# zhirui-gao/Curve-Gaussian

Hardware: AMD Instinct MI355X
Metric: Msplats rasterized/s (fwd+bwd) (higher is better)
Workload: dtype f32

## Files before the change

curve_gaussian_amd/csrc/api.hip:

```cpp
#include <math.h>
#include <stdarg.h>
#include <stdio.h>
#include <string.h>
#include <stdlib.h>

#include <algorithm>
#include <atomic>
#include <map>
#include <mutex>
#include <string>
#include <vector>

#include "kernels.h"

namespace cgs {

static thread_local char g_err[512] = "";
void set_error(const char* fmt, ...) {
    va_list ap;
    va_start(ap, fmt);
    vsnprintf(g_err, sizeof(g_err), fmt, ap);
    va_end(ap);
}

// ... 310 lines not shown
}
static void slot_abandon(int i) {
    if (g_slots[i].in_flight) (void)hipEventSynchronize(g_slots[i].ev);
    g_slots[i].in_flight = false;
    slot_release(i);
}
static bool slot_read(int i, const uint32_t* words, hipStream_t s, const char* what) {
    hipError_t e = hipMemcpyAsync(g_slots[i].h, words, 4 * sizeof(uint32_t), hipMemcpyDeviceToHost, s);
    if (e == hipSuccess) e = hipEventRecord(g_slots[i].ev, s);
    g_slots[i].in_flight = true;
    if (e != hipSuccess) set_error("%s: status readback failed: %s", what, hipGetErrorString(e));
    return e == hipSuccess;
}
static bool slot_sync(int i, const char* what) {
    const hipError_t e = hipEventSynchronize(g_slots[i].ev);
    g_slots[i].in_flight = e != hipSuccess;
    if (e != hipSuccess) set_error("%s: status readback failed: %s", what, hipGetErrorString(e));
    return e == hipSuccess;
}
static bool slot_wait(int i, const char* what) {
    if (!slot_sync(i, what)) return false;
    const StatSlot& v = g_slots[i];
    const uint32_t longest = v.h[1];
    hints_update(v.P, v.W, v.H, (uint64_t)longest <= v.cap ? (int64_t)v.h[0] : -1, longest, (int64_t)v.h[3], v.dev);
    g_last_stats[0] = (int64_t)v.h[0]; g_last_stats[1] = (int64_t)longest; g_last_stats[2] = 1;
    g_last_visible = (int64_t)v.h[2];
    return true;
}

static bool bucket_tail(hipStream_t s, const char* what, const Frame& f, const States& b, uint64_t cap, int P, const int* radii,
                        const BinHints& hints, int cull, uint32_t* nonunit, bool geo, bool unit, bool tag,
                        const float* background, float* out_color, float* out_invdepth, float* out_all_map,
                        float* color_clamped, float* dir_out, const float* wv, int slot) {
    launch_scatter_bucket(s, P, radii, b.geom.rec, f.gx, f.gy, b.img.tile_count, b.bin.keys, (uint32_t)cap, cull, b.img.total + 3,
                          hints.big > 0 ? b.img.tile_cursor : nullptr, (uint32_t)f.tiles, nonunit, scatter_spw(hints));
    if (slot >= 0) {
        uint32_t* const stat = b.img.work + 4;
        hipLaunchKernelGGL(k_count_stats, dim3(STAT_BLOCKS), dim3(256), 0, s, b.img.tile_count, f.tiles, radii, P, b.img.total + 3,
                           stat, b.img.work + VIS_COUNT_WORD);
        if (!slot_read(slot, stat, s, what)) return false;
        StatSlot& v = g_slots[slot];
        v.P = P; v.W = f.W; v.H = f.H; v.cap = cap;
    }
    if (render_fwd_can_sort((uint32_t)cap) && fuse_sort()) {
        launch_render_fwd_sorting(s, geo, f.tiles, b.img.tile_count, b.bin.keys, (uint32_t)cap, b.img.ranges, b.img.total,
                                  b.bin.point_list, f.W, f.H, f.gx, b.geom.rec, b.img.final_T, b.img.n_contrib, background,
                                  out_color, out_invdepth, out_all_map, unit, tag, color_clamped, dir_out, wv);
    } else {
        launch_tile_sort_bucket(s, f.tiles, b.img.tile_count, b.img.ranges, b.img.total, b.bin.keys, b.bin.point_list,
                                (uint32_t)cap);
        launch_render_fwd(s, geo, f.tiles, b.img.ranges, b.bin.point_list, f.W, f.H, f.gx, b.geom.rec, b.img.final_T,
                          b.img.n_contrib, background, out_color, out_invdepth, out_all_map, unit, tag);
        if (color_clamped || dir_out)
            hipLaunchKernelGGL(k_render_epilogue, dim3((unsigned)std::min<size_t>((f.npix + 255) / 256, 4096)), dim3(256), 0, s,
                               f.npix, out_color, out_all_map, wv, 1, color_clamped, dir_out);
    }
    return check_launch(what, false, s);
}

extern "C" {

const char* cgs_last_error(void) { return g_err; }
int cgs_version(void) { return 100; }
const char* cgs_target_arch(void) { return "gfx950"; }

size_t cgs_geometry_bytes(int P) {
    char* c = nullptr;
    geom_from_chunk(c, (size_t)(P > 0 ? P : 1));
    return (size_t)c + 128;
}
size_t cgs_image_bytes(int width, int height) {
    char* c = nullptr;
    const Frame f(width, height);
    image_from_chunk(c, f.npix, (size_t)f.tiles);
    return (size_t)c + 128;
}
size_t cgs_binning_bytes(int64_t R) {
    char* c = nullptr;
    bin_from_chunk(c, (size_t)(R > 0 ? R : 1));
// ... 875 lines not shown
```

curve_gaussian_amd/csrc/binning.hip:

```cpp
#include "kernels.h"

namespace cgs {

__global__ void __launch_bounds__(1024) k_scan_tiles(int tiles, const uint32_t* __restrict__ tile_count,
                                                     uint2* __restrict__ ranges, uint32_t* __restrict__ total) {
    __shared__ uint32_t wave_tot[16];
    __shared__ uint32_t wave_max[16];
    __shared__ uint32_t carry_s;
    const int tid = threadIdx.x, lane = tid & 63, wid = tid >> 6;
    if (tid == 0) carry_s = 0;
    __syncthreads();
    uint32_t vmax = 0;
    for (int base = 0; base < tiles; base += 1024) {
        const int i = base + tid;
        const uint32_t v = (i < tiles) ? tile_count[i] : 0u;
        vmax = max(vmax, v);
        uint32_t s = v;
#pragma unroll
        for (int off = 1; off < 64; off <<= 1) {
            const uint32_t n = __shfl_up(s, off, 64);
            if (lane >= off) s += n;
        }
        if (lane == 63) wave_tot[wid] = s;
        __syncthreads();
// ... 172 lines not shown
        }
        const bool gvalid = src < 64;
        const SplatWalk sp = me.fetch(gvalid ? src : lane);
        const uint32_t nt = gvalid ? sp.nt : 0u;
        for (uint32_t base = 0; __ballot(base < nt) != 0ull; base += 16) {
            const uint32_t t = base + (uint32_t)sub;
            bool pass = false;
            uint32_t tile = 0, gx_ = 0, gy_ = 0;
            if (t < nt) {
                const uint32_t ty = t / sp.w, tx = t - ty * sp.w;
                const uint32_t gxx = sp.x0 + tx, gyy = sp.y0 + ty;
                pass = !cull || tile_reach_det(sp.cx, sp.cy, sp.A, sp.B, sp.C, sp.tau2, (float)(gxx * TILE), (float)(gyy * TILE));
                tile = gyy * (uint32_t)grid_x + gxx;
                gx_ = gxx; gy_ = gyy;
            }
            fn(pass, tile, ((uint64_t)sp.khi << 32) | sp.klo, gx_, gy_);
        }
    }
}
__device__ __forceinline__ void wave_lds_fence() {
    __builtin_amdgcn_fence(__ATOMIC_RELEASE, "wavefront");
    __builtin_amdgcn_wave_barrier();
    __builtin_amdgcn_fence(__ATOMIC_ACQUIRE, "wavefront");
}
constexpr uint32_t BIG_TILES = 96;
constexpr uint32_t GW_WIN = 16, GW_CELLS = GW_WIN * GW_WIN;
#ifndef CGS_GW_LCAP
#define CGS_GW_LCAP 192
#endif
constexpr uint32_t GW_LCAP = CGS_GW_LCAP;
template <int GW_SPW>
__global__ void __launch_bounds__(256) k_scatter_window(int P, const int* __restrict__ radii,
                                                        const SplatRec* __restrict__ rec, int grid_x, int grid_y,
                                                        uint32_t* __restrict__ tile_count, uint64_t* __restrict__ keys,
                                                        uint32_t cap, int cull, uint32_t* __restrict__ big_count,
                                                        uint32_t* __restrict__ big_queue, uint32_t big_cap,
                                                        uint32_t* __restrict__ nonunit) {
    __shared__ uint32_t s_cell[4][GW_CELLS];
    __shared__ uint16_t s_ent[4][GW_LCAP];
    __shared__ uint64_t s_key[4][GW_LCAP];
    const uint32_t lane = threadIdx.x & 63, wave = threadIdx.x >> 6;
    uint32_t* wcell = s_cell[wave];
    uint16_t* went = s_ent[wave];
    uint64_t* wkey = s_key[wave];
    const int idx = (blockIdx.x * 4 + (int)wave) * GW_SPW + (int)lane;
    SplatWalk me = load_splat_walk((int)lane < GW_SPW, idx, P, radii, rec, grid_x, grid_y);
    if (nonunit && me.nonunit) *nonunit = 1u;
    if (me.nt > BIG_TILES) {
        const uint32_t q = atomicAdd(big_count, 1u);
        if (big_queue && q < big_cap) {
            big_queue[q] = (uint32_t)idx;
            me.nt = 0u;
        }
    }
    if (__ballot(me.nt > 0) == 0ull) return;
    uint32_t wx0 = me.nt > 0 ? me.x0 : 0xFFFFFFFFu, wy0 = me.nt > 0 ? me.y0 : 0xFFFFFFFFu;
#pragma unroll
    for (int off = 32; off >= 1; off >>= 1) {
        wx0 = min(wx0, (uint32_t)__shfl_xor((int)wx0, off, 64));
        wy0 = min(wy0, (uint32_t)__shfl_xor((int)wy0, off, 64));
    }
    wx0 = (uint32_t)__builtin_amdgcn_readfirstlane((int)wx0);
    wy0 = (uint32_t)__builtin_amdgcn_readfirstlane((int)wy0);
#pragma unroll
    for (uint32_t q = 0; q < GW_CELLS / 64; q++) wcell[lane + 64 * q] = 0u;
    wave_lds_fence();
    uint32_t cnt = 0;
    quad_walk(me, grid_x, cull, [&](bool pass, uint32_t tile, uint64_t key, uint32_t gxx, uint32_t gyy) {
        const uint32_t dx = gxx - wx0, dy = gyy - wy0;
        const bool inwin = pass && dx < GW_WIN && dy < GW_WIN;
        const uint64_t bal = __ballot(inwin);
        const uint32_t pos = cnt + __builtin_amdgcn_mbcnt_hi((uint32_t)(bal >> 32), __builtin_amdgcn_mbcnt_lo((uint32_t)bal, 0u));
        if (inwin && pos < GW_LCAP) {
            const uint32_t cell = dy * GW_WIN + dx;
            const uint32_t r = atomicAdd(&wcell[cell], 1u);
            went[pos] = (uint16_t)(cell | (r << 8));
            wkey[pos] = key;
        } else if (pass) {
            const uint32_t slot = atomicAdd(&tile_count[tile], 1u);
            if (slot < cap) keys[(size_t)tile * cap + slot] = key;
        }
        cnt += (uint32_t)__builtin_popcountll(bal);
    });
    const uint32_t n = min(cnt, GW_LCAP);
    if (n == 0) return;
    wave_lds_fence();
#pragma unroll
    for (uint32_t q = 0; q < GW_CELLS / 64; q++) {
        const uint32_t cell = lane + 64 * q;
        const uint32_t c = wcell[cell];
        if (c) {
            const uint32_t tile = (wy0 + cell / GW_WIN) * (uint32_t)grid_x + wx0 + cell % GW_WIN;
            wcell[cell] = atomicAdd(&tile_count[tile], c);
        }
    }
    wave_lds_fence();
    for (uint32_t j = lane; j < n; j += 64) {
        const uint32_t e = went[j], cell = e & 255u;
        const uint32_t slot = wcell[cell] + (e >> 8);
        const uint32_t tile = (wy0 + cell / GW_WIN) * (uint32_t)grid_x + wx0 + cell % GW_WIN;
        if (slot < cap) keys[(size_t)tile * cap + slot] = wkey[j];
    }
}

__global__ void __launch_bounds__(256) k_scatter_big(const uint32_t* __restrict__ big_count,
                                                     const uint32_t* __restrict__ big_queue, uint32_t big_cap,
                                                     const int* __restrict__ radii, const SplatRec* __restrict__ rec,
                                                     int grid_x, int grid_y, uint32_t* __restrict__ tile_count,
                                                     uint64_t* __restrict__ keys, uint32_t cap, int cull) {
    const uint32_t n = min(*big_count, big_cap);
    for (uint32_t e = blockIdx.x; e < n; e += gridDim.x) {
        const int idx = (int)big_queue[e];
        const float4 a = rec[idx].a;
        const float4 d = rec[idx].d;
        const float C = rec[idx].b.x;
        uint2 rmin, rmax;
        get_rect(a.x, a.y, radii[idx], grid_x, grid_y, rmin, rmax);
        const uint32_t w = max(rmax.x - rmin.x, 1u), nt = (rmax.x - rmin.x) * (rmax.y - rmin.y);
        const uint64_t key = ((uint64_t)__float_as_uint(d.x) << 32) | (uint32_t)idx;
        for (uint32_t t = threadIdx.x; t < nt; t += 256) {
            const uint32_t ty = t / w, tx = t - ty * w;
            const uint32_t gxx = rmin.x + tx, gyy = rmin.y + ty;
            if (cull && !tile_reach_det(a.x, a.y, a.z, a.w, C, d.z, (float)(gxx * TILE), (float)(gyy * TILE))) continue;
            const uint32_t tile = gyy * (uint32_t)grid_x + gxx;
            const uint32_t slot = atomicAdd(&tile_count[tile], 1u);
            if (slot < cap) keys[(size_t)tile * cap + slot] = key;
        }
    }
}

#ifndef CGS_RANK_SPLIT
#define CGS_RANK_SPLIT 1024
#endif
constexpr uint32_t RANK_SPLIT = CGS_RANK_SPLIT;
constexpr uint32_t RANK_MAX2 = 2048;
template <bool BUCKET, int KPT, bool PUBLISH>
__global__ void __launch_bounds__(256) k_tile_rank_sort(const uint2* __restrict__ ranges,
                                                        const uint64_t* __restrict__ keys,
                                                        uint32_t* __restrict__ point_list, uint32_t cap,
                                                        const uint32_t* __restrict__ tile_count,
                                                        uint2* __restrict__ ranges_out, uint32_t* __restrict__ total,
                                                        uint32_t min_n) {
    __shared__ __attribute__((aligned(16))) uint32_t sd[256 * KPT + RANK_U];
    __shared__ uint32_t si[256 * KPT];
    __shared__ uint32_t s_hist[RANK_NB], s_start[RANK_NB + 1], s_mm[8];
    const uint2 rg = BUCKET ? bucket_range(tile_count, ranges_out, total, cap, PUBLISH) : ranges[blockIdx.x];
    const uint32_t n = rg.y - rg.x;
    if (n <= min_n || n > 256u * KPT || n > (KPT == 4 ? RANK_SPLIT : ~0u) || (!BUCKET && rg.y > cap)) return;
    const uint32_t tid = threadIdx.x;
    if ((tid & ~63u) >= n) return;
    uint32_t rank[KPT], idx[KPT];
    tile_rank_sort<KPT>(keys + rg.x, n, RankScratch{sd, si, s_hist, s_start, s_mm}, rank, idx);
    uint32_t* out = point_list + rg.x;
#pragma unroll
    for (int q = 0; q < KPT; q++) {
        const uint32_t i = tid + 256u * q;
        if (i < n) out[rank[q]] = idx[q];
    }
}
// ... 30 lines not shown


void launch_scan_tiles(hipStream_t s, int tiles, const uint32_t* tile_count, uint2* ranges, uint32_t* total) {
    ProfScope p("scan_tiles", s);
    hipLaunchKernelGGL(k_scan_tiles, dim3(1), dim3(1024), 0, s, tiles, tile_count, ranges, total);
}
void launch_scatter(hipStream_t s, int P, const int* radii, const SplatRec* rec, int grid_x, int grid_y,
                    const uint2* ranges, uint32_t* tile_cursor, uint64_t* keys, uint32_t cap, int cull, uint32_t* nonunit) {
    ProfScope p("scatter", s);
    hipLaunchKernelGGL(k_scatter<false>, dim3((P + 4 * SCATTER_SPW - 1) / (4 * SCATTER_SPW)), dim3(256), 0, s, P,
                       radii, rec, grid_x, grid_y, ranges, tile_cursor, keys, cap, cull, nonunit);
}
void launch_tile_sort_small(hipStream_t s, int tiles, const uint2* ranges, uint64_t* keys, uint32_t* point_list,
                            uint32_t cap) {
    ProfScope p("tile_sort", s);
    hipLaunchKernelGGL((k_tile_rank_sort<false, 4, false>), dim3(tiles), dim3(256), 0, s, ranges, keys, point_list, cap,
                       nullptr, nullptr, nullptr, 0u);
}
void launch_tile_sort_big(hipStream_t s, int tiles, const uint2* ranges, uint64_t* keys, uint32_t* point_list,
                          uint32_t max_count) {
    if (max_count <= RANK_SPLIT) return;
    uint32_t done = RANK_SPLIT;
    if (RANK_SPLIT == RANK_MAX) {
        ProfScope p("tile_sort_mid", s);
        hipLaunchKernelGGL((k_tile_rank_sort<false, 8, false>), dim3(tiles), dim3(256), 0, s, ranges, keys, point_list,
                           ~0u, nullptr, nullptr, nullptr, RANK_MAX);
        done = RANK_MAX2;
    }
    ProfScope p("tile_sort_big", s);
    if (max_count > done)
        hipLaunchKernelGGL(k_tile_sort<false>, dim3(tiles), dim3(256), 0, s, ranges, keys, point_list, done, 0u, nullptr);
}
void launch_scatter_bucket(hipStream_t s, int P, const int* radii, const SplatRec* rec, int grid_x, int grid_y,
                           uint32_t* tile_count, uint64_t* keys, uint32_t cap, int cull, uint32_t* big_count,
                           uint32_t* big_queue, uint32_t big_cap, uint32_t* nonunit, int splats_per_wave) {
    ProfScope p("scatter", s);
    if (splats_per_wave == 8)
        hipLaunchKernelGGL(k_scatter_window<8>, dim3((P + 4 * 8 - 1) / (4 * 8)), dim3(256), 0, s, P, radii, rec, grid_x,
                           grid_y, tile_count, keys, cap, cull, big_count, big_queue, big_cap, nonunit);
    else
        hipLaunchKernelGGL(k_scatter_window<12>, dim3((P + 4 * 12 - 1) / (4 * 12)), dim3(256), 0, s, P, radii, rec, grid_x,
                           grid_y, tile_count, keys, cap, cull, big_count, big_queue, big_cap, nonunit);
    if (big_queue)
        hipLaunchKernelGGL(k_scatter_big, dim3(512), dim3(256), 0, s, big_count, big_queue, big_cap, radii, rec, grid_x,
                           grid_y, tile_count, keys, cap, cull);
}
void launch_tile_sort_bucket(hipStream_t s, int tiles, const uint32_t* tile_count, uint2* ranges, uint32_t* total,
                             uint64_t* keys, uint32_t* point_list, uint32_t cap) {
    {
        ProfScope p("tile_sort", s);
        hipLaunchKernelGGL((k_tile_rank_sort<true, 4, true>), dim3(tiles), dim3(256), 0, s, nullptr, keys, point_list, cap,
                           tile_count, ranges, total, 0u);
    }
    if (cap > RANK_SPLIT) {
        uint32_t done = RANK_SPLIT;
        if (RANK_SPLIT == RANK_MAX) {
            ProfScope p("tile_sort_mid", s);
            hipLaunchKernelGGL((k_tile_rank_sort<true, 8, false>), dim3(tiles), dim3(256), 0, s, nullptr, keys, point_list,
                               cap, tile_count, nullptr, nullptr, RANK_MAX);
            done = RANK_MAX2;
        }
        ProfScope p("tile_sort_big", s);
        if (cap > done)
            hipLaunchKernelGGL(k_tile_sort<true>, dim3(tiles), dim3(256), 0, s, nullptr, keys, point_list, done, cap,
                               tile_count);
    }
}
uint32_t bucket_cap_limit() { return SORT_LDS_KEYS; }

}
```

curve_gaussian_amd/csrc/common.h:

```cpp
#pragma once
#include <hip/hip_runtime.h>
#include <stdint.h>

#include "../../include/curvegs.h"

namespace cgs {

constexpr int TILE = 16;
constexpr int TILE_PIX = TILE * TILE;
constexpr int NUM_ALL_MAP = 4;

struct __attribute__((aligned(64))) SplatRec {
    float4 a, b, c, d;
};

constexpr int ACC_STRIDE = 16;
constexpr int ACC_STRIDE_VIEW = 8;
constexpr int ACC_COL = 6, ACC_INVD = 7, ACC_MAP = 8;

constexpr uint32_t LIST_TAG_SHIFT = 28u;
constexpr uint32_t LIST_ID_MASK = (1u << LIST_TAG_SHIFT) - 1u;

struct GeomState {
    SplatRec* rec;
    float* grad_acc;
    float* rgb;
    uint8_t* clamped;
};
constexpr int WORK_WORDS = 64 * 32;
constexpr int TOTAL_PARTS = 256;
constexpr int TOTAL_WORDS = 4 + 2 * TOTAL_PARTS;
struct ImageState {
    float* final_T;
    uint32_t* n_contrib;
    uint2* ranges;
    uint32_t* tile_count;
    uint32_t* tile_cursor;
    uint32_t* work;
    uint32_t* total;
};
struct BinState {
    uint64_t* keys;
    uint32_t* point_list;
};

template <typename T>
static inline void carve(char*& chunk, T*& ptr, size_t count) {
    uintptr_t off = (reinterpret_cast<uintptr_t>(chunk) + 127) & ~uintptr_t(127);
    ptr = reinterpret_cast<T*>(off);
    chunk = reinterpret_cast<char*>(ptr + count);
}
static inline GeomState geom_from_chunk(char*& chunk, size_t P) {
    GeomState g;
    carve(chunk, g.rec, P);
    carve(chunk, g.grad_acc, P * ACC_STRIDE);
    carve(chunk, g.rgb, P);
    carve(chunk, g.clamped, P);
    return g;
}
static inline ImageState image_from_chunk(char*& chunk, size_t npix, size_t tiles) {
    ImageState s;
    carve(chunk, s.final_T, npix);
    carve(chunk, s.n_contrib, npix);
    carve(chunk, s.ranges, tiles);
    carve(chunk, s.tile_count, tiles);
    carve(chunk, s.tile_cursor, tiles);
    carve(chunk, s.work, WORK_WORDS);
    carve(chunk, s.total, TOTAL_WORDS + 32);
    return s;
}
static inline BinState bin_from_chunk(char*& chunk, size_t R) {
    BinState b;
    carve(chunk, b.point_list, R);
    carve(chunk, b.keys, R);
    return b;
}

#ifdef __HIPCC__
__device__ __forceinline__ float3 xform4x3(const float3 p, const float* __restrict__ m) {
#pragma clang fp contract(off)
    return make_float3(m[0] * p.x + m[4] * p.y + m[8] * p.z + m[12], m[1] * p.x + m[5] * p.y + m[9] * p.z + m[13],
                       m[2] * p.x + m[6] * p.y + m[10] * p.z + m[14]);
}
__device__ __forceinline__ float4 xform4x4(const float3 p, const float* __restrict__ m) {
#pragma clang fp contract(off)
    return make_float4(m[0] * p.x + m[4] * p.y + m[8] * p.z + m[12], m[1] * p.x + m[5] * p.y + m[9] * p.z + m[13],
                       m[2] * p.x + m[6] * p.y + m[10] * p.z + m[14], m[3] * p.x + m[7] * p.y + m[11] * p.z + m[15]);
}
__device__ __forceinline__ float ndc2pix(float v, int S) { return (float)((((double)v + 1.0) * (double)S - 1.0) * 0.5); }

__device__ __forceinline__ void get_rect(float px, float py, int max_radius, int gx, int gy, uint2& rmin, uint2& rmax) {
    rmin.x = (uint32_t)min(gx, max(0, (int)((px - (float)max_radius) / (float)TILE)));
    rmin.y = (uint32_t)min(gy, max(0, (int)((py - (float)max_radius) / (float)TILE)));
    rmax.x = (uint32_t)min(gx, max(0, (int)((px + (float)max_radius + (float)(TILE - 1)) / (float)TILE)));
    rmax.y = (uint32_t)min(gy, max(0, (int)((py + (float)max_radius + (float)(TILE - 1)) / (float)TILE)));
}

__device__ __forceinline__ void quat_rows(const float4 q, float R[3][3]) {
#pragma clang fp contract(off)
    const float r = q.x, x = q.y, y = q.z, z = q.w;
// ... 119 lines not shown
#pragma unroll
        for (int q = 0; q < NQ; q++)
#pragma unroll
            for (uint32_t e = 0; e < RANK_U; e++) rank[q] += (uint32_t)(k[e] < mine[q]);
#pragma unroll
        for (uint32_t e = 0; e < RANK_U; e++) k[e] = p[e];
    }
#pragma unroll
    for (int q = 0; q < NQ; q++)
#pragma unroll
        for (uint32_t e = 0; e < RANK_U; e++) rank[q] += (uint32_t)(k[e] < mine[q]);
}
__device__ __forceinline__ uint32_t rank_loop_f32(const float* s, uint32_t n, float mine) {
    float big = 0x1p64f, nbig = -0x1p64f;
    asm volatile("" : "+v"(big), "+v"(nbig));
    const float mb = mine * big;
    const uint32_t nu = (n + 3u) & ~3u;
    float r0 = 0.f, r1 = 0.f, r2 = 0.f, r3 = 0.f;
    float4 k = *reinterpret_cast<const float4*>(s);
    for (uint32_t u = 4; u < nu; u += 4) {
        const float4 p = *reinterpret_cast<const float4*>(s + u);
        r0 += __builtin_amdgcn_fmed3f(fmaf(k.x, nbig, mb), 0.f, 1.f);
        r1 += __builtin_amdgcn_fmed3f(fmaf(k.y, nbig, mb), 0.f, 1.f);
        r2 += __builtin_amdgcn_fmed3f(fmaf(k.z, nbig, mb), 0.f, 1.f);
        r3 += __builtin_amdgcn_fmed3f(fmaf(k.w, nbig, mb), 0.f, 1.f);
        k = p;
    }
    r0 += __builtin_amdgcn_fmed3f(fmaf(k.x, nbig, mb), 0.f, 1.f);
    r1 += __builtin_amdgcn_fmed3f(fmaf(k.y, nbig, mb), 0.f, 1.f);
    r2 += __builtin_amdgcn_fmed3f(fmaf(k.z, nbig, mb), 0.f, 1.f);
    r3 += __builtin_amdgcn_fmed3f(fmaf(k.w, nbig, mb), 0.f, 1.f);
    return (uint32_t)((r0 + r1) + (r2 + r3));
}
template <typename K>
__device__ __forceinline__ void rank_dispatch(int nq, const K* s, uint32_t n, const K (&mine)[4], uint32_t (&rank)[4]) {
    switch (nq) {
        case 1: rank_loop<1>(s, n, mine, rank); break;
        case 2: rank_loop<2>(s, n, mine, rank); break;
        case 3: rank_loop<3>(s, n, mine, rank); break;
        default: rank_loop<4>(s, n, mine, rank); break;
    }
}

#ifndef CGS_RANK_PARTITION_MIN
#define CGS_RANK_PARTITION_MIN 192
#endif
constexpr uint32_t RANK_PARTITION_MIN = CGS_RANK_PARTITION_MIN;
#ifndef CGS_RANK_NB
#define CGS_RANK_NB 64
#endif
constexpr uint32_t RANK_NB = CGS_RANK_NB;
struct RankScratch {
    uint32_t* sd;
    uint32_t* si;
    uint32_t* hist;
    uint32_t* start;
    uint32_t* mm;
};
template <int KPT>
__device__ __forceinline__ void tile_rank_sort(const uint64_t* __restrict__ gk, uint32_t n, const RankScratch S,
                                               uint32_t (&rank)[KPT], uint32_t (&idx)[KPT]) {
    const uint32_t tid = threadIdx.x;
    const int lane = (int)(tid & 63u), wave = (int)(tid >> 6);
    const bool has_keys = ((uint32_t)__builtin_amdgcn_readfirstlane((int)tid) & ~63u) < n;
    const int nq = (int)((n + 255u) / 256u);
    (void)nq;
// ... 144 lines not shown
```

curve_gaussian_amd/csrc/kernels.h:

```cpp
#pragma once
#include "common.h"

namespace cgs {

void launch_preprocess_fwd(hipStream_t s, int P, int D, int M, const float* means3D, const float* scales,
                           float scale_modifier, const float* rotations, const float* opacities, const float* shs,
                           uint8_t* clamped, const float* cov3D_precomp, const float* colors_precomp,
                           const float* all_map, const float* viewmatrix, const float* projmatrix,
                           const float* cam_pos, int W, int H, float tan_fovx, float tan_fovy, float focal_x,
                           float focal_y, int* radii, SplatRec* rec, float* rgb, int grid_x, int grid_y,
                           uint32_t* tile_count, int antialiasing, int cull, float* grad_acc, uint32_t* clear_words,
                           size_t n_clear);
void launch_mark_visible(hipStream_t s, int P, const float* means3D, const float* viewmatrix, uint8_t* present);
void launch_preprocess_bwd(hipStream_t s, int P, int D, int M, const float* means3D, const int* radii,
                           const float* shs, const uint8_t* clamped, const float* opacities, const float* scales,
                           const float* rotations, float scale_modifier, const float* cov3D_precomp,
                           const float* viewmatrix, const float* projmatrix, const float* cam_pos, float focal_x,
                           float focal_y, float tan_fovx, float tan_fovy, int W, int H, const SplatRec* rec,
                           float* grad_acc, float* dL_dmean2D, float* dL_dconic, float* dL_dinvdepth,
                           float* dL_dopacity, float* dL_dmean3D, float* dL_dcolor, float* dL_dall_map,
                           float* dL_dcov3D, float* dL_dsh, float* dL_dscale, float* dL_drot, int antialiasing);

void launch_scan_tiles(hipStream_t s, int tiles, const uint32_t* tile_count, uint2* ranges, uint32_t* total);
void launch_scatter(hipStream_t s, int P, const int* radii, const SplatRec* rec, int grid_x, int grid_y,
                    const uint2* ranges, uint32_t* tile_cursor, uint64_t* keys, uint32_t cap, int cull,
                    uint32_t* nonunit = nullptr);
void launch_scatter_bucket(hipStream_t s, int P, const int* radii, const SplatRec* rec, int grid_x, int grid_y,
                           uint32_t* tile_count, uint64_t* keys, uint32_t cap, int cull, uint32_t* big_count,
                           uint32_t* big_queue, uint32_t big_cap, uint32_t* nonunit = nullptr,
                           int splats_per_wave = 12);
void launch_tile_sort_bucket(hipStream_t s, int tiles, const uint32_t* tile_count, uint2* ranges, uint32_t* total,
                             uint64_t* keys, uint32_t* point_list, uint32_t cap);
uint32_t bucket_cap_limit();
void launch_tile_sort_small(hipStream_t s, int tiles, const uint2* ranges, uint64_t* keys, uint32_t* point_list,
                            uint32_t cap);
void launch_tile_sort_big(hipStream_t s, int tiles, const uint2* ranges, uint64_t* keys, uint32_t* point_list,
                          uint32_t max_count);

void launch_render_fwd(hipStream_t s, bool geo, int tiles, const uint2* ranges, const uint32_t* point_list, int W,
                       int H, int grid_x, const SplatRec* rec, float* final_T, uint32_t* n_contrib,
                       const float* bg_color, float* out_color, float* out_invdepth, float* out_all_map,
                       bool unit = false,
                       bool tag = false);
bool render_fwd_can_sort(uint32_t cap);
void launch_render_fwd_sorting(hipStream_t s, bool geo, int tiles, const uint32_t* tile_count, const uint64_t* keys,
                               uint32_t cap, uint2* ranges, uint32_t* total, uint32_t* point_list, int W, int H,
                               int grid_x, const SplatRec* rec, float* final_T, uint32_t* n_contrib,
                               const float* bg_color, float* out_color, float* out_invdepth, float* out_all_map,
                               bool unit = false, bool tag = false,
                               float* color_clamped = nullptr, float* dir_out = nullptr, const float* wv = nullptr);
void launch_render_bwd(hipStream_t s, bool geo, bool invd, bool colg, int tiles, const uint2* ranges,
                       const uint32_t* point_list, int W, int H, int grid_x, const float* bg_color,
                       const SplatRec* rec, const float* final_Ts, const uint32_t* n_contrib, const float* dL_dpixels,
                       const float* dL_dout_invdepth, const float* dL_dout_all_map, float* grad_acc,
                       int acc_stride = ACC_STRIDE,
                       uint32_t id_mask = 0xffffffffu,
                       const uint32_t* nonunit_gate = nullptr);


void launch_render_bwd_unit(hipStream_t s, int tiles, const uint2* ranges, const uint32_t* point_list, int W, int H,
                            int grid_x, const float* bg_color, const SplatRec* rec, const float* final_Ts,
                            const uint32_t* n_contrib, const float* dL_dpixels, float* grad_acc,
                            int acc_stride = ACC_STRIDE_VIEW, const uint32_t* nonunit_gate = nullptr,
                            const float* clamp_raw = nullptr);

int sample_norm_words();
void launch_sample_norms(hipStream_t s, int B, int m, const float* cp, const uint8_t* is_bezier, const void* coef, double* norms);
void launch_sample_backward_close(hipStream_t s, int B, int m, const float* cp, const float* width, const uint8_t* is_bezier,
                                  const void* coef, float eps, const double* norms, const float* part, float* g_cp, float* g_width,
                                  int accumulate);
void launch_view_forward(hipStream_t s, int B, int m, const float* cp, const float* width, const uint8_t* is_bezier,
                         const void* coef, float eps, const double* norms, const float* opacity_logit,
                         const float* mask_logit, float mask_thr, const float* colors_precomp, const float* campos,
                         const float* viewmatrix, const float* projmatrix, float tan_fovx, float tan_fovy, float focal_x,
                         float focal_y, int W, int H, int grid_x, int grid_y, float* xyz, float* rot, float* scl, int* radii,
                         SplatRec* rec, float* grad_acc, uint32_t* clear_words, size_t n_clear);
void launch_view_backward(hipStream_t s, int B, int m, const float* cp, const float* width, const uint8_t* is_bezier,
                          const void* coef, float eps, double* norms, const float* opacity_logit, const float* mask_logit,
// ... 60 lines not shown
```

curve_gaussian_amd/csrc/render.hip:

```cpp
#include "kernels.h"
#include "p2_mfma.h"
#include "composite.h"

namespace cgs {

constexpr int BATCH = 256;
__device__ __forceinline__ float sat01(float x) { return __builtin_amdgcn_fmed3f(x, 0.f, 1.f); }
struct StepConsts {
    float big, cA;
};
__device__ __forceinline__ StepConsts step_consts() {
    StepConsts k;
    k.big = 0x1p100f;
    k.cA = -__uint_as_float(0x3b808080u) * 0x1p100f;
    asm volatile("" : "+v"(k.big), "+v"(k.cA));
    return k;
}
constexpr int SLOTS = 8;

struct BucketSort {
    const uint32_t* tile_count;
    const uint64_t* keys;
    uint32_t* point_list;
    uint2* ranges;
    uint32_t* total;
    uint32_t cap;
};

struct ViewEpilogue {
    float* color_clamped;
    float* dir_out;
    const float* wv;
};

constexpr int GROUP = 16;
#ifndef CGS_WHATIF
#define CGS_WHATIF 0
#endif
#ifndef CGS_FWD3_WAVES
#define CGS_FWD3_WAVES 6
#endif
#ifndef CGS_FWD3_WAVES_GENERAL
#define CGS_FWD3_WAVES_GENERAL CGS_FWD3_WAVES
#endif
#ifndef CGS_FWD_FAST
#define CGS_FWD_FAST 1
#endif
#ifndef CGS_BWD3_WHATIF
#define CGS_BWD3_WHATIF 0
#endif
#ifndef CGS_BWD3_WAVES
#define CGS_BWD3_WAVES 6
#endif
#ifndef CGS_BWD3_CAP
#define CGS_BWD3_CAP 104
#endif
constexpr int BWD_BATCH = 128;
static_assert(CGS_BWD3_CAP % 8 == 0 && CGS_BWD3_CAP <= BWD_BATCH, "CGS_BWD3_CAP: a multiple of SLOTS (8), at most BWD_BATCH");
constexpr uint32_t BWD_PAD_OFF = (BWD_BATCH + 1) * 16;
constexpr uint32_t PAD_OFF = (BATCH + 1) * 16;

template <bool GEO, bool SORT, bool UNIT = false, bool TAG = UNIT>
__global__ void __launch_bounds__(256, UNIT ? CGS_FWD3_WAVES : CGS_FWD3_WAVES_GENERAL) k_render_fwd3(const uint2* __restrict__ ranges,
                                                     const uint32_t* __restrict__ point_list, int W, int H, int grid_x,
                                                     const SplatRec* __restrict__ rec, float* __restrict__ final_T,
                                                     uint32_t* __restrict__ n_contrib, const float* __restrict__ bg_color,
                                                     float* __restrict__ out_color, float* __restrict__ out_invdepth,
                                                     float* __restrict__ out_all_map, BucketSort bs, ViewEpilogue epi) {
    constexpr bool IMAGE_ONLY = UNIT && !GEO;
    __shared__ float4 s_geo[BATCH + 2];
    __shared__ float4 s_at[BATCH + 2];
    __shared__ float4 s_c[GEO ? BATCH + 2 : 1];
    __shared__ uint64_t s_qmask[4][4];
    __shared__ __attribute__((aligned(16))) uint32_t s_list[4][BATCH + GROUP];
    __shared__ __attribute__((aligned(16))) uint32_t s_ord[SORT ? RANK_MAX + RANK_U : 1];
    __shared__ uint32_t s_si[SORT ? RANK_MAX : 1];
    __shared__ uint32_t s_hist[SORT ? RANK_NB : 1], s_start[SORT ? RANK_NB + 1 : 1], s_mm[8];
    if (threadIdx.x == 0) {
        s_geo[BATCH + 1] = make_float4(0.f, 0.f, 0.f, 0.f);
        s_at[BATCH + 1] = make_float4(0.f, 0.f, 0.f, L2_NEVER);
        if (GEO) s_c[GEO ? BATCH + 1 : 0] = make_float4(0.f, 0.f, 0.f, 0.f);
    }
    const TileGeom g = tile_geom(W, H, grid_x);
    const int lane = g.lane;
    const float X0 = (float)(g.tx * TILE), Y0 = (float)(g.ty * TILE);
    uint2 range;
    bool prestaged = false;
    if (SORT) {
        const uint32_t tid = threadIdx.x;
        const uint32_t base = g.tile * bs.cap;
        uint64_t key0 = ~0ull;
        if (CGS_FWD_FAST && tid < bs.cap) key0 = bs.keys[base + tid];
        const uint32_t cnt = bs.tile_count[g.tile];
        const uint32_t n = min(cnt, bs.cap);
        range = make_uint2(base, base + n);
        if (tid == 0) {
            bs.ranges[g.tile] = range;
            if (cnt) {
                uint32_t* part = bs.total + 4 + 2 * (g.tile % TOTAL_PARTS);
                atomicAdd(&part[0], n);
                atomicMax(&part[1], cnt);
                if (cnt > bs.cap) {
                    bs.total[2] = 1u;
                    atomicAdd(&bs.total[TOTAL_WORDS], 1u);
                }
            }
        }
        if (CGS_FWD_FAST && n > 0 && n <= (uint32_t)BATCH) {
            const bool has = tid < n;
            const uint32_t depth = has ? (uint32_t)(key0 >> 32) : ~0u;
            const uint32_t id = has ? (uint32_t)key0 : 0u;
            const SplatRec* r = rec + id;
            float4 ra = make_float4(0.f, 0.f, 1.f, 0.f), rb = make_float4(1.f, 0.f, 0.f, 0.f), rc = ra;
            float tau2 = -1.f;
            if (has && !(CGS_WHATIF & 256)) {
                ra = r->a;
                rb = r->b;
                if (GEO) rc = r->c;
                tau2 = r->d.z;
            }
            if (has) s_ord[tid] = depth;
            if (tid < 4u) s_ord[n + tid] = 0x7f800000u;
            s_si[tid] = 0u;
            __syncthreads();
            uint32_t lost = 0u;
            if (((uint32_t)__builtin_amdgcn_readfirstlane((int)tid) & ~63u) < n) {
                const uint32_t rk[1] = {(CGS_WHATIF & 32) ? tid : rank_loop_f32(reinterpret_cast<const float*>(s_ord), n, __uint_as_float(depth))};
                if (has) {
                    float4 sa, sb;
                    stage_splat(ra, rb, sa, sb);
                    const uint32_t slot = rk[0] + 1u;
                    s_geo[slot] = sa;
                    s_at[slot] = make_float4(sb.z, sb.w, sb.x, __builtin_amdgcn_logf(sb.y));
                    if (GEO) s_c[GEO ? slot : 0] = UNIT ? make_float4(rc.x, rc.y, rc.z, sb.w) : rc;
                    const uint32_t qm = (CGS_WHATIF & 128) ? 15u : quadrant_mask(ra, rb, tau2, X0, Y0);
                    lost = atomicExch(&s_si[rk[0]], 0x100u | qm);
                    bs.point_list[base + rk[0]] = TAG ? (id | (qm << LIST_TAG_SHIFT)) : id;
                }
            }
            prestaged = !__syncthreads_or((int)lost);
        }
        if (n > 0 && !prestaged) {
            uint32_t rank[4], idx[4];
            tile_rank_sort<4>(bs.keys + base, n, RankScratch{s_ord, s_si, s_hist, s_start, s_mm}, rank, idx);
#pragma unroll
            for (int q = 0; q < 4; q++) {
                const uint32_t i = tid + 256u * q;
                if (i < n) {
                    s_ord[rank[q]] = idx[q];
                    if (!TAG || rank[q] >= (uint32_t)BATCH) bs.point_list[base + rank[q]] = idx[q];
                }
            }
            __syncthreads();
        }
    } else {
        range = ranges[g.tile];
    }
    const int total = (int)(range.y - range.x);
    const int rounds = (total + BATCH - 1) / BATCH;
    const StepConsts k = step_consts();
    float T_dead = 0.0f;
    float Tw = 1.0f;
    float cA = g.inside ? k.cA : -0x1p126f;
    uint32_t last_contributor = 0;
    float C = 0.f, Dacc = 0.f;
    float A0 = 0.f, A1 = 0.f, A2 = 0.f, A3 = 0.f;
    bool wave_done = ballot64(cA > -0x1p120f) == 0ull;
    const P2Frag pix = p2_pixel_operand(lane);
    const int row_splat = p2_row_splat(lane);
    const float hx = X0 + (float)((g.wave & 1) << 3) + 3.5f;
// ... 484 lines not shown
#pragma unroll
                        for (int w = 0; w < 4; w++) {
                            const uint64_t m = tm[w][c];
                            const int pos = base[w][c] + __builtin_popcountll(m & ((1ull << bit) - 1ull));
                            if (((m >> bit) & 1ull) && pos < CAP) { v += s_res[w][pos * NF + f]; any = true; }
                        }
                        if (any && v != 0.f) {
                            const uint32_t id = INVD ? s_id[e + 1] : __float_as_uint(s_at[e + 1].y);
                            atomicAdd(grad_acc + (size_t)id * acc_stride + f, v);
                        }
                    }
                }
            }
        }
    }
}

#define CGS_FWD3(G, S, U, T, R, PL, BS)                                                                               \
    hipLaunchKernelGGL((k_render_fwd3<G, S, U, T>), dim3(tiles), dim3(256), 0, s, R, PL, W, H, grid_x, rec, final_T,  \
                       n_contrib, bg_color, out_color, out_invdepth, out_all_map, BS, epi)
void launch_render_fwd(hipStream_t s, bool geo, int tiles, const uint2* ranges, const uint32_t* point_list, int W,
                       int H, int grid_x, const SplatRec* rec, float* final_T, uint32_t* n_contrib,
                       const float* bg_color, float* out_color, float* out_invdepth, float* out_all_map, bool unit, bool tag) {
    ProfScope p("render_fwd", s);
    const ViewEpilogue epi{nullptr, nullptr, nullptr};
    if (geo && unit) CGS_FWD3(true, false, true, true, ranges, point_list, BucketSort{});
    else if (unit) CGS_FWD3(false, false, true, true, ranges, point_list, BucketSort{});
    else if (geo && tag) CGS_FWD3(true, false, false, true, ranges, point_list, BucketSort{});
    else if (tag) CGS_FWD3(false, false, false, true, ranges, point_list, BucketSort{});
    else if (geo) CGS_FWD3(true, false, false, false, ranges, point_list, BucketSort{});
    else CGS_FWD3(false, false, false, false, ranges, point_list, BucketSort{});
}
bool render_fwd_can_sort(uint32_t cap) { return cap <= RANK_MAX; }
void launch_render_fwd_sorting(hipStream_t s, bool geo, int tiles, const uint32_t* tile_count, const uint64_t* keys,
                               uint32_t cap, uint2* ranges, uint32_t* total, uint32_t* point_list, int W, int H,
                               int grid_x, const SplatRec* rec, float* final_T, uint32_t* n_contrib,
                               const float* bg_color, float* out_color, float* out_invdepth, float* out_all_map, bool unit,
                               bool tag, float* color_clamped, float* dir_out, const float* wv) {
    ProfScope p("render_fwd", s);
    const BucketSort bs{tile_count, keys, point_list, ranges, total, cap};
    const ViewEpilogue epi{color_clamped, geo ? dir_out : nullptr, wv};
    const uint2* no_ranges = nullptr;
    const uint32_t* no_list = nullptr;
    if (geo && unit) CGS_FWD3(true, true, true, true, no_ranges, no_list, bs);
    else if (unit) CGS_FWD3(false, true, true, true, no_ranges, no_list, bs);
    else if (geo && tag) CGS_FWD3(true, true, false, true, no_ranges, no_list, bs);
    else if (tag) CGS_FWD3(false, true, false, true, no_ranges, no_list, bs);
    else if (geo) CGS_FWD3(true, true, false, false, no_ranges, no_list, bs);
    else CGS_FWD3(false, true, false, false, no_ranges, no_list, bs);
}
#undef CGS_FWD3
void launch_render_bwd(hipStream_t s, bool geo, bool invd, bool colg, int tiles, const uint2* ranges,
                       const uint32_t* point_list, int W, int H, int grid_x, const float* bg_color,
                       const SplatRec* rec, const float* final_Ts, const uint32_t* n_contrib, const float* dL_dpixels,
                       const float* dL_dout_invdepth, const float* dL_dout_all_map, float* grad_acc, int acc_stride,
                       uint32_t id_mask, const uint32_t* nonunit_gate) {
    ProfScope p("render_bwd", s);
#define CGS_BWD(G, I, C)                                                                                         \
    hipLaunchKernelGGL((k_render_bwd3<G, I, C>), dim3(tiles), dim3(256), 0, s, ranges, point_list, W, H, grid_x, \
                       bg_color, rec, final_Ts, n_contrib, dL_dpixels, dL_dout_invdepth, dL_dout_all_map, grad_acc, acc_stride, id_mask, nonunit_gate)
    if (geo && invd) CGS_BWD(true, true, true);
    else if (geo) CGS_BWD(true, false, true);
    else if (invd) CGS_BWD(false, true, true);
    else if (colg) CGS_BWD(false, false, true);
    else CGS_BWD(false, false, false);
#undef CGS_BWD
}

}
```

Measured before the change: 817.7.

## Bucket per-tile depth ranking into sub-ranges using scatter-tracked depth bounds

```diff
diff --git a/curve_gaussian_amd/csrc/api.hip b/curve_gaussian_amd/csrc/api.hip
--- a/curve_gaussian_amd/csrc/api.hip
+++ b/curve_gaussian_amd/csrc/api.hip
@@ -366,8 +366,9 @@
                         const BinHints& hints, int cull, uint32_t* nonunit, bool geo, bool unit, bool tag,
                         const float* background, float* out_color, float* out_invdepth, float* out_all_map,
                         float* color_clamped, float* dir_out, const float* wv, int slot) {
-    launch_scatter_bucket(s, P, radii, b.geom.rec, f.gx, f.gy, b.img.tile_count, b.bin.keys, (uint32_t)cap, cull, b.img.total + 3,
-                          hints.big > 0 ? b.img.tile_cursor : nullptr, (uint32_t)f.tiles, nonunit, scatter_spw(hints));
+    launch_scatter_bucket(s, P, radii, b.geom.rec, f.gx, f.gy, b.img.tile_count, b.img.tile_depth, b.bin.keys, (uint32_t)cap, cull,
+                          b.img.total + 3, hints.big > 0 ? b.img.tile_cursor : nullptr, (uint32_t)f.tiles, nonunit,
+                          scatter_spw(hints));
     if (slot >= 0) {
         uint32_t* const stat = b.img.work + 4;
         hipLaunchKernelGGL(k_count_stats, dim3(STAT_BLOCKS), dim3(256), 0, s, b.img.tile_count, f.tiles, radii, P, b.img.total + 3,
@@ -377,8 +378,8 @@
         v.P = P; v.W = f.W; v.H = f.H; v.cap = cap;
     }
     if (render_fwd_can_sort((uint32_t)cap) && fuse_sort()) {
-        launch_render_fwd_sorting(s, geo, f.tiles, b.img.tile_count, b.bin.keys, (uint32_t)cap, b.img.ranges, b.img.total,
-                                  b.bin.point_list, f.W, f.H, f.gx, b.geom.rec, b.img.final_T, b.img.n_contrib, background,
+        launch_render_fwd_sorting(s, geo, f.tiles, b.img.tile_count, b.img.tile_depth, b.bin.keys, (uint32_t)cap, b.img.ranges,
+                                  b.img.total, b.bin.point_list, f.W, f.H, f.gx, b.geom.rec, b.img.final_T, b.img.n_contrib, background,
                                   out_color, out_invdepth, out_all_map, unit, tag, color_clamped, dir_out, wv);
     } else {
         launch_tile_sort_bucket(s, f.tiles, b.img.tile_count, b.img.ranges, b.img.total, b.bin.keys, b.bin.point_list,
diff --git a/curve_gaussian_amd/csrc/binning.hip b/curve_gaussian_amd/csrc/binning.hip
--- a/curve_gaussian_amd/csrc/binning.hip
+++ b/curve_gaussian_amd/csrc/binning.hip
@@ -228,10 +228,10 @@
 template <int GW_SPW>
 __global__ void __launch_bounds__(256) k_scatter_window(int P, const int* __restrict__ radii,
                                                         const SplatRec* __restrict__ rec, int grid_x, int grid_y,
-                                                        uint32_t* __restrict__ tile_count, uint64_t* __restrict__ keys,
-                                                        uint32_t cap, int cull, uint32_t* __restrict__ big_count,
-                                                        uint32_t* __restrict__ big_queue, uint32_t big_cap,
-                                                        uint32_t* __restrict__ nonunit) {
+                                                        uint32_t* __restrict__ tile_count, uint2* __restrict__ tile_depth,
+                                                        uint64_t* __restrict__ keys, uint32_t cap, int cull,
+                                                        uint32_t* __restrict__ big_count, uint32_t* __restrict__ big_queue,
+                                                        uint32_t big_cap, uint32_t* __restrict__ nonunit) {
     __shared__ uint32_t s_cell[4][GW_CELLS];
     __shared__ uint16_t s_ent[4][GW_LCAP];
     __shared__ uint64_t s_key[4][GW_LCAP];
@@ -251,13 +251,18 @@
     }
     if (__ballot(me.nt > 0) == 0ull) return;
     uint32_t wx0 = me.nt > 0 ? me.x0 : 0xFFFFFFFFu, wy0 = me.nt > 0 ? me.y0 : 0xFFFFFFFFu;
+    uint32_t wlo = me.nt > 0 ? ~me.khi : 0u, whi = me.nt > 0 ? me.khi : 0u;
 #pragma unroll
     for (int off = 32; off >= 1; off >>= 1) {
         wx0 = min(wx0, (uint32_t)__shfl_xor((int)wx0, off, 64));
         wy0 = min(wy0, (uint32_t)__shfl_xor((int)wy0, off, 64));
+        wlo = max(wlo, (uint32_t)__shfl_xor((int)wlo, off, 64));
+        whi = max(whi, (uint32_t)__shfl_xor((int)whi, off, 64));
     }
     wx0 = (uint32_t)__builtin_amdgcn_readfirstlane((int)wx0);
     wy0 = (uint32_t)__builtin_amdgcn_readfirstlane((int)wy0);
+    wlo = (uint32_t)__builtin_amdgcn_readfirstlane((int)wlo);
+    whi = (uint32_t)__builtin_amdgcn_readfirstlane((int)whi);
 #pragma unroll
     for (uint32_t q = 0; q < GW_CELLS / 64; q++) wcell[lane + 64 * q] = 0u;
     wave_lds_fence();
@@ -275,6 +280,8 @@
         } else if (pass) {
             const uint32_t slot = atomicAdd(&tile_count[tile], 1u);
             if (slot < cap) keys[(size_t)tile * cap + slot] = key;
+            atomicMax(&tile_depth[tile].x, ~(uint32_t)(key >> 32));
+            atomicMax(&tile_depth[tile].y, (uint32_t)(key >> 32));
         }
         cnt += (uint32_t)__builtin_popcountll(bal);
     });
@@ -288,6 +295,8 @@
         if (c) {
             const uint32_t tile = (wy0 + cell / GW_WIN) * (uint32_t)grid_x + wx0 + cell % GW_WIN;
             wcell[cell] = atomicAdd(&tile_count[tile], c);
+            atomicMax(&tile_depth[tile].x, wlo);
+            atomicMax(&tile_depth[tile].y, whi);
         }
     }
     wave_lds_fence();
@@ -303,7 +312,8 @@
                                                      const uint32_t* __restrict__ big_queue, uint32_t big_cap,
                                                      const int* __restrict__ radii, const SplatRec* __restrict__ rec,
                                                      int grid_x, int grid_y, uint32_t* __restrict__ tile_count,
-                                                     uint64_t* __restrict__ keys, uint32_t cap, int cull) {
+                                                     uint2* __restrict__ tile_depth, uint64_t* __restrict__ keys,
+                                                     uint32_t cap, int cull) {
     const uint32_t n = min(*big_count, big_cap);
     for (uint32_t e = blockIdx.x; e < n; e += gridDim.x) {
         const int idx = (int)big_queue[e];
@@ -321,6 +331,8 @@
             const uint32_t tile = gyy * (uint32_t)grid_x + gxx;
             const uint32_t slot = atomicAdd(&tile_count[tile], 1u);
             if (slot < cap) keys[(size_t)tile * cap + slot] = key;
+            atomicMax(&tile_depth[tile].x, ~__float_as_uint(d.x));
+            atomicMax(&tile_depth[tile].y, __float_as_uint(d.x));
         }
     }
 }
@@ -417,18 +429,20 @@
         hipLaunchKernelGGL(k_tile_sort<false>, dim3(tiles), dim3(256), 0, s, ranges, keys, point_list, done, 0u, nullptr);
 }
 void launch_scatter_bucket(hipStream_t s, int P, const int* radii, const SplatRec* rec, int grid_x, int grid_y,
-                           uint32_t* tile_count, uint64_t* keys, uint32_t cap, int cull, uint32_t* big_count,
-                           uint32_t* big_queue, uint32_t big_cap, uint32_t* nonunit, int splats_per_wave) {
+                           uint32_t* tile_count, uint32_t* tile_depth, uint64_t* keys, uint32_t cap, int cull,
+                           uint32_t* big_count, uint32_t* big_queue, uint32_t big_cap, uint32_t* nonunit,
+                           int splats_per_wave) {
     ProfScope p("scatter", s);
+    uint2* const depth = reinterpret_cast<uint2*>(tile_depth);
     if (splats_per_wave == 8)
         hipLaunchKernelGGL(k_scatter_window<8>, dim3((P + 4 * 8 - 1) / (4 * 8)), dim3(256), 0, s, P, radii, rec, grid_x,
-                           grid_y, tile_count, keys, cap, cull, big_count, big_queue, big_cap, nonunit);
+                           grid_y, tile_count, depth, keys, cap, cull, big_count, big_queue, big_cap, nonunit);
     else
         hipLaunchKernelGGL(k_scatter_window<12>, dim3((P + 4 * 12 - 1) / (4 * 12)), dim3(256), 0, s, P, radii, rec, grid_x,
-                           grid_y, tile_count, keys, cap, cull, big_count, big_queue, big_cap, nonunit);
+                           grid_y, tile_count, depth, keys, cap, cull, big_count, big_queue, big_cap, nonunit);
     if (big_queue)
         hipLaunchKernelGGL(k_scatter_big, dim3(512), dim3(256), 0, s, big_count, big_queue, big_cap, radii, rec, grid_x,
-                           grid_y, tile_count, keys, cap, cull);
+                           grid_y, tile_count, depth, keys, cap, cull);
 }
 void launch_tile_sort_bucket(hipStream_t s, int tiles, const uint32_t* tile_count, uint2* ranges, uint32_t* total,
                              uint64_t* keys, uint32_t* point_list, uint32_t cap) {
diff --git a/curve_gaussian_amd/csrc/common.h b/curve_gaussian_amd/csrc/common.h
--- a/curve_gaussian_amd/csrc/common.h
+++ b/curve_gaussian_amd/csrc/common.h
@@ -37,6 +37,7 @@
     uint32_t* tile_count;
     uint32_t* tile_cursor;
     uint32_t* work;
+    uint32_t* tile_depth;
     uint32_t* total;
 };
 struct BinState {
@@ -66,6 +67,7 @@
     carve(chunk, s.tile_count, tiles);
     carve(chunk, s.tile_cursor, tiles);
     carve(chunk, s.work, WORK_WORDS);
+    carve(chunk, s.tile_depth, 2 * tiles);
     carve(chunk, s.total, TOTAL_WORDS + 32);
     return s;
 }
@@ -251,6 +253,19 @@
     r3 += __builtin_amdgcn_fmed3f(fmaf(k.w, nbig, mb), 0.f, 1.f);
     return (uint32_t)((r0 + r1) + (r2 + r3));
 }
+__device__ __forceinline__ uint32_t rank_slice_f32(const float* s, uint32_t len, float mine) {
+    float big = 0x1p64f, nbig = -0x1p64f;
+    asm volatile("" : "+v"(big), "+v"(nbig));
+    const float mb = mine * big;
+    float r0 = 0.f, r1 = 0.f, r2 = 0.f, r3 = 0.f;
+    for (uint32_t u = 0; u < len; u += 4) {
+        r0 += __builtin_amdgcn_fmed3f(fmaf(s[u], nbig, mb), 0.f, 1.f);
+        r1 += __builtin_amdgcn_fmed3f(fmaf(s[u + 1], nbig, mb), 0.f, 1.f);
+        r2 += __builtin_amdgcn_fmed3f(fmaf(s[u + 2], nbig, mb), 0.f, 1.f);
+        r3 += __builtin_amdgcn_fmed3f(fmaf(s[u + 3], nbig, mb), 0.f, 1.f);
+    }
+    return (uint32_t)((r0 + r1) + (r2 + r3));
+}
 template <typename K>
 __device__ __forceinline__ void rank_dispatch(int nq, const K* s, uint32_t n, const K (&mine)[4], uint32_t (&rank)[4]) {
     switch (nq) {
diff --git a/curve_gaussian_amd/csrc/kernels.h b/curve_gaussian_amd/csrc/kernels.h
--- a/curve_gaussian_amd/csrc/kernels.h
+++ b/curve_gaussian_amd/csrc/kernels.h
@@ -26,8 +26,8 @@
                     const uint2* ranges, uint32_t* tile_cursor, uint64_t* keys, uint32_t cap, int cull,
                     uint32_t* nonunit = nullptr);
 void launch_scatter_bucket(hipStream_t s, int P, const int* radii, const SplatRec* rec, int grid_x, int grid_y,
-                           uint32_t* tile_count, uint64_t* keys, uint32_t cap, int cull, uint32_t* big_count,
-                           uint32_t* big_queue, uint32_t big_cap, uint32_t* nonunit = nullptr,
+                           uint32_t* tile_count, uint32_t* tile_depth, uint64_t* keys, uint32_t cap, int cull,
+                           uint32_t* big_count, uint32_t* big_queue, uint32_t big_cap, uint32_t* nonunit = nullptr,
                            int splats_per_wave = 12);
 void launch_tile_sort_bucket(hipStream_t s, int tiles, const uint32_t* tile_count, uint2* ranges, uint32_t* total,
                              uint64_t* keys, uint32_t* point_list, uint32_t cap);
@@ -43,7 +43,8 @@
                        bool unit = false,
                        bool tag = false);
 bool render_fwd_can_sort(uint32_t cap);
-void launch_render_fwd_sorting(hipStream_t s, bool geo, int tiles, const uint32_t* tile_count, const uint64_t* keys,
+void launch_render_fwd_sorting(hipStream_t s, bool geo, int tiles, const uint32_t* tile_count, const uint32_t* tile_depth,
+                               const uint64_t* keys,
                                uint32_t cap, uint2* ranges, uint32_t* total, uint32_t* point_list, int W, int H,
                                int grid_x, const SplatRec* rec, float* final_T, uint32_t* n_contrib,
                                const float* bg_color, float* out_color, float* out_invdepth, float* out_all_map,
diff --git a/curve_gaussian_amd/csrc/render.hip b/curve_gaussian_amd/csrc/render.hip
--- a/curve_gaussian_amd/csrc/render.hip
+++ b/curve_gaussian_amd/csrc/render.hip
@@ -20,6 +20,7 @@
 
 struct BucketSort {
     const uint32_t* tile_count;
+    const uint2* tile_depth;
     const uint64_t* keys;
     uint32_t* point_list;
     uint2* ranges;
@@ -46,6 +47,11 @@
 #ifndef CGS_FWD_FAST
 #define CGS_FWD_FAST 1
 #endif
+#ifndef CGS_FWD_NB
+#define CGS_FWD_NB 32
+#endif
+constexpr uint32_t FWD_NB = CGS_FWD_NB;
+static_assert(FWD_NB >= 1 && FWD_NB <= RANK_NB, "CGS_FWD_NB: 1 .. RANK_NB sub-ranges");
 #ifndef CGS_BWD3_WHATIF
 #define CGS_BWD3_WHATIF 0
 #endif
@@ -92,6 +98,7 @@
         uint64_t key0 = ~0ull;
         if (CGS_FWD_FAST && tid < bs.cap) key0 = bs.keys[base + tid];
         const uint32_t cnt = bs.tile_count[g.tile];
+        const uint2 dbound = CGS_FWD_FAST ? bs.tile_depth[g.tile] : make_uint2(0u, 0u);
         const uint32_t n = min(cnt, bs.cap);
         range = make_uint2(base, base + n);
         if (tid == 0) {
@@ -119,23 +126,50 @@
                 if (GEO) rc = r->c;
                 tau2 = r->d.z;
             }
-            if (has) s_ord[tid] = depth;
+            const uint32_t lo = min(~dbound.x, dbound.y), hi = dbound.y;
+            const float scale = (float)FWD_NB * __builtin_amdgcn_rcpf((float)(hi - lo) + 1.0f);
+            const uint32_t sub = min(FWD_NB - 1u, (uint32_t)((float)(min(max(depth, lo), hi) - lo) * scale));
+            if (tid < FWD_NB) s_hist[tid] = 0u;
             if (tid < 4u) s_ord[n + tid] = 0x7f800000u;
             s_si[tid] = 0u;
             __syncthreads();
+            uint32_t pos = 0u;
+            if (has) pos = atomicAdd(&s_hist[sub], 1u);
+            __syncthreads();
+            const bool wave_has = ((uint32_t)__builtin_amdgcn_readfirstlane((int)tid) & ~63u) < n;
+            uint32_t start = 0u, len = 0u;
+            if (wave_has) {
+                const uint32_t l = tid & 63u;
+                const uint32_t c = l < FWD_NB ? s_hist[l] : 0u;
+                uint32_t v = c;
+                v += (uint32_t)__builtin_amdgcn_update_dpp(0, (int)v, 0x111, 0xF, 0xF, true);
+                v += (uint32_t)__builtin_amdgcn_update_dpp(0, (int)v, 0x112, 0xF, 0xF, true);
+                v += (uint32_t)__builtin_amdgcn_update_dpp(0, (int)v, 0x114, 0xF, 0xF, true);
+                v += (uint32_t)__builtin_amdgcn_update_dpp(0, (int)v, 0x118, 0xF, 0xF, true);
+                const uint32_t t0 = (uint32_t)__builtin_amdgcn_readlane((int)v, 15);
+                const uint32_t t1 = (uint32_t)__builtin_amdgcn_readlane((int)v, 31);
+                const uint32_t t2 = (uint32_t)__builtin_amdgcn_readlane((int)v, 47);
+                v += (l >= 16u ? t0 : 0u) + (l >= 32u ? t1 : 0u) + (l >= 48u ? t2 : 0u);
+                start = (uint32_t)__shfl((int)(v - c), (int)sub, 64);
+                len = (uint32_t)__shfl((int)c, (int)sub, 64);
+                if (has) s_ord[start + pos] = depth;
+            }
+            __syncthreads();
             uint32_t lost = 0u;
-            if (((uint32_t)__builtin_amdgcn_readfirstlane((int)tid) & ~63u) < n) {
-                const uint32_t rk[1] = {(CGS_WHATIF & 32) ? tid : rank_loop_f32(reinterpret_cast<const float*>(s_ord), n, __uint_as_float(depth))};
+            if (wave_has) {
+                const uint32_t rk = (CGS_WHATIF & 32) ? tid
+                                    : start + rank_slice_f32(reinterpret_cast<const float*>(s_ord) + start, has ? len : 0u,
+                                                             __uint_as_float(depth));
                 if (has) {
                     float4 sa, sb;
                     stage_splat(ra, rb, sa, sb);
-                    const uint32_t slot = rk[0] + 1u;
+                    const uint32_t slot = rk + 1u;
                     s_geo[slot] = sa;
                     s_at[slot] = make_float4(sb.z, sb.w, sb.x, __builtin_amdgcn_logf(sb.y));
                     if (GEO) s_c[GEO ? slot : 0] = UNIT ? make_float4(rc.x, rc.y, rc.z, sb.w) : rc;
                     const uint32_t qm = (CGS_WHATIF & 128) ? 15u : quadrant_mask(ra, rb, tau2, X0, Y0);
-                    lost = atomicExch(&s_si[rk[0]], 0x100u | qm);
-                    bs.point_list[base + rk[0]] = TAG ? (id | (qm << LIST_TAG_SHIFT)) : id;
+                    lost = atomicExch(&s_si[rk], 0x100u | qm);
+                    bs.point_list[base + rk] = TAG ? (id | (qm << LIST_TAG_SHIFT)) : id;
                 }
             }
             prestaged = !__syncthreads_or((int)lost);
@@ -686,13 +720,13 @@
     else CGS_FWD3(false, false, false, false, ranges, point_list, BucketSort{});
 }
 bool render_fwd_can_sort(uint32_t cap) { return cap <= RANK_MAX; }
-void launch_render_fwd_sorting(hipStream_t s, bool geo, int tiles, const uint32_t* tile_count, const uint64_t* keys,
-                               uint32_t cap, uint2* ranges, uint32_t* total, uint32_t* point_list, int W, int H,
-                               int grid_x, const SplatRec* rec, float* final_T, uint32_t* n_contrib,
+void launch_render_fwd_sorting(hipStream_t s, bool geo, int tiles, const uint32_t* tile_count, const uint32_t* tile_depth,
+                               const uint64_t* keys, uint32_t cap, uint2* ranges, uint32_t* total, uint32_t* point_list, int W,
+                               int H, int grid_x, const SplatRec* rec, float* final_T, uint32_t* n_contrib,
                                const float* bg_color, float* out_color, float* out_invdepth, float* out_all_map, bool unit,
                                bool tag, float* color_clamped, float* dir_out, const float* wv) {
     ProfScope p("render_fwd", s);
-    const BucketSort bs{tile_count, keys, point_list, ranges, total, cap};
+    const BucketSort bs{tile_count, reinterpret_cast<const uint2*>(tile_depth), keys, point_list, ranges, total, cap};
     const ViewEpilogue epi{color_clamped, geo ? dir_out : nullptr, wv};
     const uint2* no_ranges = nullptr;
     const uint32_t* no_list = nullptr;
```

After: 819.2, median of 6. Within noise of the previous version (+0.2%).
